# MGI-tech-bioinformatics/SuperPlus

Hardware: AMD Instinct MI355X
Metric: k-mers/s (DF createDict stage: trim + canonical k-mer count + solid filter + spectrum + adjacency) (higher is better)
Workload: dtype u64

## Files before the change

superplus_amd/csrc/dfk.hip:

```cpp
#include "../../include/dfk.h"
#include "dfk_kernels.h"

#include <algorithm>
#include <chrono>
#include <cstdarg>
#include <cstdio>
#include <cstdlib>
#include <cstring>
#include <atomic>
#include <fcntl.h>
#include <functional>
#include <new>
#include <string>
#include <sys/mman.h>
#include <sys/stat.h>
#include <unistd.h>
#include <condition_variable>
#include <memory>
#include <mutex>
#include <thread>
#include <vector>

using namespace dfk;

// ... 276 lines not shown
template <int K>
int stage_trim(dfk_ctx* c, const Inputs& in, uint64_t* n_inst)
{
    DevBuf ctr; int rc = c->alloc(ctr, 32, "trim counters"); if (rc) return rc;
    HIP_TRY(hipMemsetAsync(ctr.p, 0, 32, c->stream));
    rc = c->alloc(c->good_len, sizeof(uint32_t) * in.n_reads, "goodLens", true); if (rc) return rc;
    if (in.n_reads) {
        unsigned grid = (unsigned)std::min<uint64_t>((in.n_reads + 255) / 256, 8192);
        hipLaunchKernelGGL(HIP_KERNEL_NAME(k_trim<K>), dim3(grid), dim3(256), 0, c->stream,
                           in.pq, in.pq_off, in.pq_bytes, in.base_off, in.packed_bytes, in.read_len, in.n_reads, c->cfg.min_qual, (uint32_t*)c->good_len.p,
                           (unsigned long long*)ctr.p, (unsigned int*)((char*)ctr.p + 8),
                           (unsigned long long*)((char*)ctr.p + 16));
        HIP_TRY(hipGetLastError());
    }
    uint64_t h[3] = {0, 0, 0};
    HIP_TRY(hipMemcpyAsync(h, ctr.p, 24, hipMemcpyDeviceToHost, c->stream));
    HIP_TRY(hipStreamSynchronize(c->stream));
    c->release(ctr);
    if ((uint32_t)h[1]) return fail(DFK_E_INPUT, "malformed input: an offset table is not monotone or runs past its array, a PQVec stream is broken, or its length differs from read_len");
    if (h[2] == 0) return fail(DFK_E_NOGOOD, "Looks like your input data have almost no good bases.");
    *n_inst = h[0];
    return 0;
}

int device_scan(dfk_ctx* c, const uint64_t* in, uint64_t* out, uint64_t n)
{
    constexpr uint64_t PER = (uint64_t)SCAN_THREADS * SCAN_ITEMS;
    if (n == 0) return 0;
    const uint64_t nblk = (n + PER - 1) / PER;
    if (nblk == 1) {
        hipLaunchKernelGGL(k_scan_blocks, dim3(1), dim3(SCAN_THREADS), 0, c->stream, in, out, n, (uint64_t*)nullptr);
        HIP_TRY(hipGetLastError());
        return 0;
    }
    DevBuf sums; int rc = c->alloc(sums, nblk * 8, "scan block sums"); if (rc) return rc;
    hipLaunchKernelGGL(k_scan_blocks, dim3((unsigned)nblk), dim3(SCAN_THREADS), 0, c->stream, in, out, n, (uint64_t*)sums.p);
    HIP_TRY(hipGetLastError());
    rc = device_scan(c, (const uint64_t*)sums.p, (uint64_t*)sums.p, nblk); if (rc) return rc;
    hipLaunchKernelGGL(k_scan_add, dim3((unsigned)nblk), dim3(SCAN_THREADS), 0, c->stream, out, n, (const uint64_t*)sums.p);
    HIP_TRY(hipGetLastError());
    HIP_TRY(hipStreamSynchronize(c->stream));
    c->release(sums);
    return 0;
}

struct BucketTable {
    uint32_t log2_nb = 0;
    DevBuf acc;
    DevBuf summ;
    DevBuf classes;
    DevBuf ovf_list; uint64_t n_ovf = 0;
    DevBuf class_hist;
    std::vector<uint64_t> h_class;
    uint64_t n_records = 0, n_inst = 0;
};
struct Partition {
    DevBuf records, base, ipre, items;
    uint64_t n_records = 0, n_inst = 0, n_items = 0;
    uint64_t nb = 0;
};

template <int K>
PartParams part_params(const dfk_ctx* c, uint32_t log2_nb, uint32_t log2_world, int64_t read_id0, uint32_t sub_lo, uint32_t sub_n)
{
    const uint32_t M = c->cfg.minimizer_len;
    return PartParams{M, (uint32_t)K - M + 1, log2_nb, log2_world, read_id0, sub_lo, sub_n,
                      sweep_class_mask(sub_lo, sub_n, log2_nb - log2_world)};
}

int table_totals(dfk_ctx* c, const DevBuf& acc, uint64_t nb, uint64_t* n_records, uint64_t* n_inst)
{
    DevBuf tot; int rc = c->alloc(tot, 16, "bucket totals"); if (rc) return rc;
    HIP_TRY(hipMemsetAsync(tot.p, 0, 16, c->stream));
    hipLaunchKernelGGL(k_sum_acc, dim3(1024), dim3(256), 0, c->stream, (const unsigned long long*)acc.p, nb, (unsigned long long*)tot.p);
    HIP_TRY(hipGetLastError());
    uint64_t h[2];
    HIP_TRY(hipMemcpyAsync(h, tot.p, 16, hipMemcpyDeviceToHost, c->stream));
    HIP_TRY(hipStreamSynchronize(c->stream));
    c->release(tot);
    *n_records = h[0]; *n_inst = h[1];
    return 0;
}

struct ScanJob {
    PartParams pp; uint64_t nb = 0, n_bins = 0, ovf_cap = 0; bool by_class = false, ranged = false;
    DevBuf ovf_tmp, d_n;
    bool keyed = false; uint32_t n_cls = 0, n_sub = 0, sb = 0; uint64_t piece_reads = 0;
    ScanKeys sk{};
    DevBuf keys, keys2, fill, sub;
    std::vector<std::pair<hipEvent_t, hipEvent_t>> ev;
    ~ScanJob() { for (auto& e : ev) { (void)hipEventDestroy(e.first); (void)hipEventDestroy(e.second); } }
};

template <int K> bool scan_takes_ranges(const dfk_ctx* c) { return c->cfg.minimizer_len == 16; }

template <int K>
int scan_begin(dfk_ctx* c, const Inputs& in, uint32_t log2_world, int64_t read_id0, BucketTable* T, bool by_class, ScanJob* J)
{
    J->pp = part_params<K>(c, T->log2_nb, log2_world, read_id0, 0, 1u << (T->log2_nb - log2_world));
    J->nb = 1ull << T->log2_nb; J->by_class = by_class;
    int rc = 0;
    J->n_bins = 2ull * (PART_CLASSES << log2_world);
    if (by_class) { rc = c->alloc(T->class_hist, J->n_bins * 8, "class counters", true); if (rc) return rc; HIP_TRY(hipMemsetAsync(T->class_hist.p, 0, J->n_bins * 8, c->stream)); }
    else { rc = c->alloc(T->acc, J->nb * 8, "bucket counters", true); if (rc) return rc; }
    rc = c->alloc(T->summ, std::max<uint64_t>(1, in.n_reads) * 16, "run summaries", true); if (rc) return rc;
    rc = c->alloc(T->classes, std::max<uint64_t>(1, in.n_reads) * 4, "read bucket classes", true); if (rc) return rc;
    if (!by_class) HIP_TRY(hipMemsetAsync(T->acc.p, 0, J->nb * 8, c->stream));
    J->ovf_cap = in.n_reads / 16 + 1024;
    rc = c->alloc(J->ovf_tmp, J->ovf_cap * 4, "overflow read list (scratch)"); if (rc) return rc;
    rc = c->alloc(J->d_n, 16, "overflow read count"); if (rc) return rc;
    HIP_TRY(hipMemsetAsync(J->d_n.p, 0, 16, c->stream));
    const double runs = in.n_reads ? 1.0 + 2.0 * std::max(0.0, 4.0 * (double)in.packed_bytes / (double)in.n_reads - K + 1) / (J->pp.W + 1) : 0.0;
    J->keyed = !by_class && scan_takes_ranges<K>(c) && in.n_reads && (runs >= 3.5 || getenv("DFK_SCAN_KEY_PIECE"));
    if (J->keyed) {
        const uint32_t lb = T->log2_nb, cb = std::min<uint32_t>(6, lb);
        J->sk.ib = lb - cb; J->n_cls = 1u << cb;
        J->sb = std::min(KEY_SUB_BITS, J->sk.ib); J->n_sub = 1u << (J->sk.ib - J->sb);
        const double per_read = 1.25 * runs;
        constexpr uint64_t KEY_SCRATCH_MAX = 16ull << 30;
        const uint64_t want = 8ull * (uint64_t)(per_read * (double)in.n_reads) + 8ull * J->n_cls;
        const uint64_t room = std::min<uint64_t>(std::min(want, KEY_SCRATCH_MAX), c->largest_allocatable() / 3);
        J->sk.cap = std::max<uint64_t>(1024, room / 8 / J->n_cls);
        J->piece_reads = std::max<uint64_t>(PART_THREADS, (uint64_t)((double)(J->sk.cap * J->n_cls) / per_read));
        if (const char* e = getenv("DFK_SCAN_KEY_PIECE")) J->piece_reads = std::max<uint64_t>(1, std::min<uint64_t>(J->piece_reads, strtoull(e, nullptr, 10)));
        const uint64_t n_subs = (uint64_t)J->n_cls * J->n_sub;
        rc = c->alloc(J->keys, J->sk.cap * J->n_cls * 4, "run keys (scratch)"); if (rc) return rc;
        rc = c->alloc(J->keys2, J->sk.cap * J->n_cls * 4, "run keys by sub-slice (scratch)"); if (rc) return rc;
        rc = c->alloc(J->fill, J->n_cls * 8, "run key slice fills (scratch)"); if (rc) return rc;
        rc = c->alloc(J->sub, (3 * n_subs + 1) * 8, "run key sub-slices (scratch)"); if (rc) return rc;
        J->sk.keys = (uint32_t*)J->keys.p; J->sk.fill = (unsigned long long*)J->fill.p;
        TRACE("run keys: %u classes of %llu keys, %u sub-slices each, pieces of %llu reads", J->n_cls, (unsigned long long)J->sk.cap,
              J->n_sub, (unsigned long long)J->piece_reads);
    }
    return 0;
}

template <int K>
int scan_keys_piece(dfk_ctx* c, const Inputs& in, BucketTable* T, ScanJob* J, uint64_t r0, uint64_t r1)
{
    static const unsigned scan_blocks = getenv("DFK_SCAN_BLOCKS") ? (unsigned)atoi(getenv("DFK_SCAN_BLOCKS")) : 0;
    const unsigned cus = (unsigned)c->prop.multiProcessorCount;
    const unsigned grid = (unsigned)std::min<uint64_t>((r1 - r0 + PART_THREADS - 1) / PART_THREADS, (uint64_t)(scan_blocks ? scan_blocks : 128u) * cus);
    const uint64_t n_subs = (uint64_t)J->n_cls * J->n_sub;
    auto* cnt = (unsigned long long*)J->sub.p;
    auto* off = cnt + n_subs;
    auto* cur = off + n_subs + 1;
    HIP_TRY(hipMemsetAsync(J->fill.p, 0, J->n_cls * 8, c->stream));
    HIP_TRY(hipMemsetAsync(cnt, 0, n_subs * 8, c->stream));
    const size_t lds = SCAN_RUN_LDS + SCAN_STAGE_LDS;
    hipLaunchKernelGGL(HIP_KERNEL_NAME(k_scan_count<K, 16, true>), dim3(grid), dim3(PART_THREADS), lds, c->stream,
                       in.packed, in.packed_bytes, in.base_off, (const uint32_t*)c->good_len.p, r0, r1, J->pp,
                       (unsigned long long*)T->acc.p, (unsigned long long*)nullptr, (unsigned long long*)J->d_n.p, J->ovf_cap,
                       (uint32_t*)J->ovf_tmp.p, (uint4*)T->summ.p, (uint32_t*)T->classes.p, J->sk);
    HIP_TRY(hipGetLastError());
    const dim3 per_class(std::max(1u, 16u * cus / J->n_cls), J->n_cls);
    const uint32_t sh = 6 + J->sb;
    hipLaunchKernelGGL(k_keys_subcount, per_class, dim3(256), J->n_sub * 4, c->stream,
                       (const uint32_t*)J->keys.p, (const unsigned long long*)J->fill.p, J->sk.cap, sh, J->n_sub, cnt);
    HIP_TRY(hipGetLastError());
    hipLaunchKernelGGL(k_keys_offsets, dim3(1), dim3(1024), 0, c->stream, (const unsigned long long*)cnt, (uint32_t)n_subs, off, cur);
    HIP_TRY(hipGetLastError());
    hipLaunchKernelGGL(k_keys_partition, per_class, dim3(256), J->n_sub * 12, c->stream,
                       (const uint32_t*)J->keys.p, (const unsigned long long*)J->fill.p, J->sk.cap, sh, J->n_sub, cur, (uint32_t*)J->keys2.p);
    HIP_TRY(hipGetLastError());
    hipLaunchKernelGGL(k_keys_count, dim3((unsigned)n_subs), dim3(1024), 0, c->stream,
                       (const uint32_t*)J->keys2.p, (const unsigned long long*)off, J->sb, (unsigned long long*)T->acc.p);
    HIP_TRY(hipGetLastError());
    return 0;
}

template <int K>
int scan_range(dfk_ctx* c, const Inputs& in, BucketTable* T, ScanJob* J, uint64_t r0, uint64_t r1)
{
    if (r1 <= r0) return 0;
    const PartParams& pp = J->pp;
    const bool by_class = J->by_class;
    unsigned grid = (unsigned)((r1 - r0 + PART_THREADS - 1) / PART_THREADS);
    static const unsigned scan_blocks = getenv("DFK_SCAN_BLOCKS") ? (unsigned)atoi(getenv("DFK_SCAN_BLOCKS")) : 0;
    if (by_class) grid = std::min<unsigned>(grid, (scan_blocks ? scan_blocks : 128u) * (unsigned)c->prop.multiProcessorCount);
    else if (scan_blocks) grid = std::min<unsigned>(grid, scan_blocks * (unsigned)c->prop.multiProcessorCount);
    const size_t lds_a = (sizeof(uint32_t) + 1) * pp.W * PART_THREADS + sizeof(uint32_t) * PART_RING * PART_THREADS + (by_class ? J->n_bins * 4 : 0);
    hipEvent_t e0, e1;
    HIP_TRY(hipEventCreate(&e0)); HIP_TRY(hipEventCreate(&e1));
    J->ev.emplace_back(e0, e1);
    HIP_TRY(hipEventRecord(e0, c->stream));
    if (J->keyed) {
        for (uint64_t p0 = r0; p0 < r1; p0 += J->piece_reads) {
            int rc = scan_keys_piece<K>(c, in, T, J, p0, std::min(r1, p0 + J->piece_reads)); if (rc) return rc;
        }
    } else if (scan_takes_ranges<K>(c)) {
        const size_t lds_r = SCAN_RUN_LDS + (by_class ? J->n_bins * 4 : 0);
        hipLaunchKernelGGL(HIP_KERNEL_NAME(k_scan_count<K, 16, false>), dim3(grid), dim3(PART_THREADS), lds_r, c->stream,
                           in.packed, in.packed_bytes, in.base_off, (const uint32_t*)c->good_len.p, r0, r1, pp,
                           (unsigned long long*)T->acc.p, (unsigned long long*)T->class_hist.p, (unsigned long long*)J->d_n.p, J->ovf_cap,
                           (uint32_t*)J->ovf_tmp.p, (uint4*)T->summ.p, (uint32_t*)T->classes.p, ScanKeys{});
    } else {
        if (r0 != 0 || r1 != in.n_reads) return fail(DFK_E_STATE, "the general scan takes every read at once");
        hipLaunchKernelGGL(HIP_KERNEL_NAME(k_partition<K, false>), dim3(grid), dim3(PART_THREADS), lds_a, c->stream,
                           in.packed, in.packed_bytes, in.base_off, (const uint32_t*)c->good_len.p, in.bc,
                           (int64_t)c->cfg.ign_bc_below, in.n_reads, pp, (unsigned long long*)T->acc.p, (unsigned long long*)T->class_hist.p,
                           (unsigned long long*)J->d_n.p, J->ovf_cap, (uint4*)J->ovf_tmp.p, (uint4*)T->summ.p,
                           (const uint32_t*)nullptr, (uint64_t)0, (const uint64_t*)nullptr, (uint32_t*)T->classes.p);
    }
    HIP_TRY(hipGetLastError());
    HIP_TRY(hipEventRecord(e1, c->stream));
    return 0;
}

template <int K>
int scan_end(dfk_ctx* c, const Inputs& in, uint64_t n_inst, BucketTable* T, ScanJob* J)
{
    int rc = 0;
    T->n_ovf = 0;
    c->release(J->keys); c->release(J->keys2); c->release(J->fill); c->release(J->sub);
    if (in.n_reads) {
        HIP_TRY(hipMemcpyAsync(&T->n_ovf, J->d_n.p, 8, hipMemcpyDeviceToHost, c->stream));
        HIP_TRY(hipStreamSynchronize(c->stream));
        if (T->n_ovf > J->ovf_cap) {
            c->release(J->ovf_tmp);
            rc = c->alloc(J->ovf_tmp, in.n_reads * 4, "overflow read list (scratch)"); if (rc) return rc;
            HIP_TRY(hipMemsetAsync(J->d_n.p, 0, 16, c->stream));
            hipLaunchKernelGGL(k_select_overflow, dim3((unsigned)std::min<uint64_t>((in.n_reads + 255) / 256, 8192)), dim3(256), 0, c->stream,
                               (const uint4*)T->summ.p, in.n_reads, (uint32_t*)J->ovf_tmp.p, (unsigned long long*)J->d_n.p);
            HIP_TRY(hipGetLastError());
            HIP_TRY(hipMemcpyAsync(&T->n_ovf, J->d_n.p, 8, hipMemcpyDeviceToHost, c->stream));
            HIP_TRY(hipStreamSynchronize(c->stream));
        }
        if (T->n_ovf) {
            rc = c->alloc(T->ovf_list, T->n_ovf * 4, "overflow read list", true); if (rc) return rc;
            HIP_TRY(hipMemcpyAsync(T->ovf_list.p, J->ovf_tmp.p, T->n_ovf * 4, hipMemcpyDeviceToDevice, c->stream));
            HIP_TRY(hipStreamSynchronize(c->stream));
        }
    }
    c->release(J->ovf_tmp); c->release(J->d_n);
    HIP_TRY(hipStreamSynchronize(c->stream));
    float ms = 0;
    for (auto& e : J->ev) { float m = 0; if (hipEventElapsedTime(&m, e.first, e.second) == hipSuccess) ms += m; }
    c->st.ms_part_count = ms; c->st.reserved[6] = J->ev.size();
    TRACE("%llu of %llu reads have more than %d runs", (unsigned long long)T->n_ovf, (unsigned long long)in.n_reads, SUMMARY_RUNS);
    if (J->by_class) {
        T->h_class.assign(J->n_bins, 0);
        HIP_TRY(hipMemcpyAsync(T->h_class.data(), T->class_hist.p, J->n_bins * 8, hipMemcpyDeviceToHost, c->stream));
        HIP_TRY(hipStreamSynchronize(c->stream));
        T->n_records = T->n_inst = 0;
        for (uint64_t i = 0; i < J->n_bins / 2; ++i) { T->n_records += T->h_class[i]; T->n_inst += T->h_class[J->n_bins / 2 + i]; }
    } else { rc = table_totals(c, T->acc, J->nb, &T->n_records, &T->n_inst); if (rc) return rc; }
    TRACE("partition count pass done (%llu buckets, %llu records%s)", (unsigned long long)J->nb, (unsigned long long)T->n_records, J->ev.size() > 1 ? ", in ranges under the upload" : "");
    if (T->n_inst != n_inst)
        return fail(DFK_E_HIP, "partition count pass saw %llu instances, trim saw %llu%s",
                    (unsigned long long)T->n_inst, (unsigned long long)n_inst,
                    (n_inst - T->n_inst) % (1ull << 32) == 0 ? " (a fine bucket with 2^32 or more instances: its counter keeps 32 bits)" : "");
    c->st.n_records = T->n_records; c->st.n_buckets = J->nb;
    return 0;
}

template <int K>
int partition_count(dfk_ctx* c, const Inputs& in, uint64_t n_inst, uint32_t log2_world, int64_t read_id0, BucketTable* T, bool by_class = false)
{
    ScanJob J;
    int rc = scan_begin<K>(c, in, log2_world, read_id0, T, by_class, &J); if (rc) return rc;
    rc = scan_range<K>(c, in, T, &J, 0, in.n_reads); if (rc) return rc;
    return scan_end<K>(c, in, n_inst, T, &J);
}

int pass_tables(dfk_ctx* c, const DevBuf& acc, uint32_t log2_sub, uint32_t world, uint32_t sub_lo, uint32_t sub_n, uint64_t budget, Partition* P)
{
    P->nb = (uint64_t)world * sub_n;
    const uint64_t nb = P->nb;
    DevBuf rec, inst, flags, idx;
    int rc = c->alloc(rec, (nb + 1) * 8, "bucket record counts"); if (rc) return rc;
    rc = c->alloc(inst, (nb + 1) * 8, "bucket instance counts"); if (rc) return rc;
    rc = c->alloc(P->base, (nb + 1) * 8, "bucket bases"); if (rc) return rc;
    rc = c->alloc(P->ipre, (nb + 1) * 8, "bucket instance prefix"); if (rc) return rc;
    const unsigned g1 = (unsigned)((nb + 1 + 255) / 256);
    hipLaunchKernelGGL(k_slice, dim3(g1), dim3(256), 0, c->stream, (const unsigned long long*)acc.p, log2_sub, sub_lo, sub_n, nb,
                       (uint64_t*)rec.p, (uint64_t*)inst.p);
    HIP_TRY(hipGetLastError());
    rc = device_scan(c, (const uint64_t*)rec.p, (uint64_t*)P->base.p, nb + 1); if (rc) return rc;
    rc = device_scan(c, (const uint64_t*)inst.p, (uint64_t*)P->ipre.p, nb + 1); if (rc) return rc;
    rc = c->alloc(flags, (nb + 1) * 8, "item flags"); if (rc) return rc;
    rc = c->alloc(idx, (nb + 1) * 8, "item index"); if (rc) return rc;
    hipLaunchKernelGGL(k_item_flags, dim3(g1), dim3(256), 0, c->stream, (const uint64_t*)P->ipre.p, nb, budget, (uint64_t*)flags.p);
    HIP_TRY(hipGetLastError());
    rc = device_scan(c, (const uint64_t*)flags.p, (uint64_t*)idx.p, nb + 1); if (rc) return rc;
    uint64_t tot[3];
    HIP_TRY(hipMemcpyAsync(&tot[0], (const uint64_t*)P->base.p + nb, 8, hipMemcpyDeviceToHost, c->stream));
    HIP_TRY(hipMemcpyAsync(&tot[1], (const uint64_t*)P->ipre.p + nb, 8, hipMemcpyDeviceToHost, c->stream));
    HIP_TRY(hipMemcpyAsync(&tot[2], (const uint64_t*)idx.p + nb, 8, hipMemcpyDeviceToHost, c->stream));
    HIP_TRY(hipStreamSynchronize(c->stream));
    P->n_records = tot[0]; P->n_inst = tot[1]; P->n_items = tot[2];
    rc = c->alloc(P->items, std::max<uint64_t>(1, P->n_items) * sizeof(ItemRange), "work items"); if (rc) return rc;
    hipLaunchKernelGGL(k_item_pairs, dim3((unsigned)((nb + 255) / 256)), dim3(256), 0, c->stream, (const uint64_t*)flags.p,
                       (const uint64_t*)idx.p, nb, (ItemRange*)P->items.p);
    HIP_TRY(hipGetLastError());
    HIP_TRY(hipStreamSynchronize(c->stream));
    c->release(rec); c->release(inst); c->release(flags); c->release(idx);
// ... 1642 lines not shown
```

superplus_amd/csrc/dfk_kernels.h:

```cpp
#pragma once
#include <type_traits>
#include "dfk_device.h"

namespace dfk {

template <int K>
__global__ void __launch_bounds__(256)
k_trim(const uint8_t* __restrict__ pq, const uint64_t* __restrict__ pq_off, uint64_t pq_nbytes,
       const uint64_t* __restrict__ base_off, uint64_t packed_bytes, const uint32_t* __restrict__ read_len,
       uint64_t n_reads, uint32_t min_qual, uint32_t* __restrict__ good_len,
       unsigned long long* __restrict__ n_inst, unsigned int* __restrict__ bad,
       unsigned long long* __restrict__ sum_good)
{
    unsigned long long mine = 0, good = 0;
    bool any_bad = false;
    for (uint64_t r = (uint64_t)blockIdx.x * blockDim.x + threadIdx.x; r < n_reads; r += (uint64_t)gridDim.x * blockDim.x) {
        uint32_t gl = 0;
        uint64_t p = pq_off[r], end = pq_off[r + 1];
        uint32_t idx = 0, run = 0;
        const uint64_t b0 = base_off[r], b1 = base_off[r + 1];
        bool ok = p <= end && end <= pq_nbytes && b0 <= b1 && b1 <= packed_bytes && b1 - b0 >= ((uint64_t)read_len[r] + 3) / 4;
        if (!ok) end = p;
        while (p < end) {
            uint32_t nQs = pq[p];
// ... 267 lines not shown
                for (int k = 0; k < 8; ++k) v[k] = i0 - k >= 0 ? arr[(i0 - k) * PART_THREADS + tid] : 0u;
#pragma unroll
                for (int k = 0; k < 8; ++k) {
                    const int i = i0 - k;
                    if (i >= 0) {
                        const bool lt = v[k] < run;
                        run = lt ? v[k] : run;
                        arr[i * PART_THREADS + tid] = run;
                        if (!WRITE) { ri = lt ? (uint32_t)i : ri; sidx[i * PART_THREADS + tid] = (uint8_t)ri; }
                    }
                }
            }
            bi = 0;
        }
        if (bi + 1 < W) sfx_next = arr[(bi + 1) * PART_THREADS + tid];
    }
    close_run();
    if (!WRITE) {
        const uint64_t lo = sum_lo | (qn <= (uint32_t)SUMMARY_RUNS ? qn : SUMMARY_OVERFLOW), hi = sum_hi;
        summaries[r] = uint4{(uint32_t)lo, (uint32_t)(lo >> 32), (uint32_t)hi, (uint32_t)(hi >> 32)};
        if (read_classes) read_classes[r] = cmask;
        if (qn > (uint32_t)SUMMARY_RUNS && bucket_cur) {
            const unsigned long long at = atomicAdd(bucket_cur, 1ull);
            if (at < n_out) reinterpret_cast<uint32_t*>(records)[at] = (uint32_t)r;
        }
    }
    if (WRITE) {
        for (uint32_t e = 0; e < qn; ++e) {
            uint32_t a = queue[(2 * e) * PART_THREADS + tid], b = queue[(2 * e + 1) * PART_THREADS + tid];
            const uint64_t dst = place(b);
            if (dst != ~0ull) emit_record<K>(words, n_words, bit0, a & 0xFFFFu, a >> 16, b, gl, tag, dst, records);
        }
    }
}

template <int K, bool WRITE>
__global__ void __launch_bounds__(PART_THREADS)
k_partition(const uint8_t* __restrict__ packed, uint64_t packed_bytes, const uint64_t* __restrict__ base_off,
            const uint32_t* __restrict__ good_len, const int32_t* __restrict__ bc, int64_t ign_bc_below,
            uint64_t n_reads, PartParams pp,
            unsigned long long* __restrict__ bucket_acc,
            unsigned long long* __restrict__ class_hist,
            unsigned long long* __restrict__ bucket_cur,
            uint64_t n_out,
            uint4* __restrict__ records,
            uint4* __restrict__ summaries,
            const uint32_t* __restrict__ read_list,
            uint64_t n_list,
            const uint64_t* __restrict__ slice_base,
            uint32_t* __restrict__ read_classes)
{
    extern __shared__ uint32_t smem[];
    uint32_t* lh = nullptr;
    const uint32_t n_bins = 2u * (PART_CLASSES << pp.log2_world);
    if (!WRITE && class_hist) {
        lh = reinterpret_cast<uint32_t*>(reinterpret_cast<uint8_t*>(smem) + 5 * pp.W * PART_THREADS + 4 * PART_RING * PART_THREADS);
        for (uint32_t i = threadIdx.x; i < n_bins; i += PART_THREADS) lh[i] = 0;
        __syncthreads();
    }
    const uint64_t n_work = (WRITE && read_list) ? n_list : n_reads;
    for (uint64_t r0 = (uint64_t)blockIdx.x * PART_THREADS; r0 < n_work; r0 += (uint64_t)gridDim.x * PART_THREADS)
        partition_read<K, WRITE>(r0 + threadIdx.x, smem, lh, packed, packed_bytes, base_off, good_len, bc, ign_bc_below, n_reads, pp,
                                 bucket_acc, bucket_cur, n_out, records, summaries, read_list, n_list, slice_base, read_classes);
    if (lh) {
        __syncthreads();
        for (uint32_t i = threadIdx.x; i < n_bins; i += PART_THREADS) if (lh[i]) atomicAdd(&class_hist[i], (unsigned long long)lh[i]);
    }
}

template <int I, int N, class F>
__device__ __forceinline__ void static_for(F&& f)
{
    if constexpr (I < N) { f(std::integral_constant<int, I>{}); static_for<I + 1, N>(f); }
}

struct ScanKeys {
    uint32_t* keys;
    unsigned long long* fill;
    uint64_t cap;
    uint32_t ib;
};
constexpr int SCAN_STAGE = 1536;
constexpr uint32_t KEY_SUB_BITS = 14;
constexpr uint32_t KEY_TILE = 16384;

template <int K, int M, bool KEYS>
__global__ void __launch_bounds__(PART_THREADS)
k_scan_count(const uint8_t* __restrict__ packed, uint64_t packed_bytes, const uint64_t* __restrict__ base_off,
             const uint32_t* __restrict__ good_len, uint64_t r_first, uint64_t n_reads , PartParams pp,
             unsigned long long* __restrict__ bucket_acc, unsigned long long* __restrict__ class_hist,
             unsigned long long* __restrict__ ovf_count, uint64_t ovf_cap, uint32_t* __restrict__ ovf_list,
             uint4* __restrict__ summaries, uint32_t* __restrict__ read_classes, ScanKeys sk)
{
    constexpr int W = K - M + 1;
    constexpr uint32_t mmask = M == 16 ? 0xFFFFFFFFu : ((1u << (2 * M)) - 1u);
    constexpr uint32_t rsh = 2 * (M - 1);
    constexpr int RUNS = SUMMARY_RUNS;
    static_assert(KTraits<K>::NK_MAX < 64, "nk takes the key's six low bits");
    extern __shared__ uint32_t smem[];
    uint32_t* runb = smem;
    uint16_t* runf = reinterpret_cast<uint16_t*>(runb + RUNS * PART_THREADS);
    uint32_t* const after_runs = reinterpret_cast<uint32_t*>(runf + RUNS * PART_THREADS);
    uint32_t* lh = nullptr;
    const uint32_t n_bins = 2u * (PART_CLASSES << pp.log2_world);
    if (class_hist) {
        lh = after_runs;
        for (uint32_t i = threadIdx.x; i < n_bins; i += PART_THREADS) lh[i] = 0;
        __syncthreads();
    }
    const int tid = threadIdx.x;
    uint32_t* st_key = after_runs;
    unsigned long long* st_base = reinterpret_cast<unsigned long long*>(st_key + SCAN_STAGE);
    uint32_t* st_h = reinterpret_cast<uint32_t*>(st_base + PART_CLASSES);
    uint32_t* st_n = st_h + PART_CLASSES;
    uint8_t* st_cls = reinterpret_cast<uint8_t*>(st_n + 1);
    const uint32_t n_cls = 1u << (pp.log2_nb - sk.ib);
    if constexpr (KEYS) {
        if (tid < PART_CLASSES) st_h[tid] = 0;
        if (tid == 0) *st_n = 0;
        __syncthreads();
    }
    auto flush = [&]() {
        const uint32_t n = *st_n;
        if (tid < (int)n_cls) { const uint32_t h = st_h[tid]; if (h) st_base[tid] = atomicAdd(&sk.fill[tid], (unsigned long long)h); st_h[tid] = 0; }
        __syncthreads();
        for (uint32_t j = tid; j < n; j += PART_THREADS) {
            const uint32_t key = st_key[j], cls = st_cls[j];
            const unsigned long long at = st_base[cls] + atomicAdd(&st_h[cls], 1u);
            if (at < sk.cap) sk.keys[cls * sk.cap + at] = key;
            else atomicAdd(&bucket_acc[(cls << sk.ib) | (key >> 6)], (1ull << 32) | (key & 63u));
        }
        __syncthreads();
        if (tid < (int)n_cls) st_h[tid] = 0;
        if (tid == 0) *st_n = 0;
        __syncthreads();
    };
    const uint32_t* words = reinterpret_cast<const uint32_t*>(packed);
    const uint64_t n_words = (packed_bytes + 3) >> 2;
    const uint32_t log2_local = pp.log2_nb - pp.log2_world;
    for (uint64_t r0 = r_first + (uint64_t)blockIdx.x * PART_THREADS; r0 < n_reads; r0 += (uint64_t)gridDim.x * PART_THREADS) {
        const uint64_t r = r0 + tid;
        const uint32_t gl = r < n_reads ? good_len[r] : 0;
        const bool live = gl >= (uint32_t)K + 1;
        uint32_t qn = 0, cmask = 0;
        uint64_t sum_lo = 0, sum_hi = 0;
        if (live) {
            const uint64_t bit0 = base_off[r] * 8;
            constexpr int NW = (2 * W + 30 + 31) / 32, NA = (2 * W + 31) / 32;
            auto load = [&](uint64_t bit, uint32_t (&w)[NW]) {
                const uint64_t wi = bit >> 5;
#pragma unroll
                for (int k = 0; k < NW; ++k) {
                    const uint64_t i = wi + k;
                    const uint32_t v = words[i < n_words ? i : n_words - 1];
                    w[k] = i < n_words ? v : 0u;
                }
            };
            uint64_t nbit = bit0 + 2 * (M - 1);
            uint32_t nw[NW];
            load(nbit, nw);
            uint32_t f = 0, rc = 0;
            {
                const uint64_t wi = bit0 >> 5;
                const uint32_t w0 = words[wi < n_words ? wi : n_words - 1], w1 = words[wi + 1 < n_words ? wi + 1 : n_words - 1];
                const uint32_t pw = alignbit(wi + 1 < n_words ? w1 : 0u, wi < n_words ? w0 : 0u, (uint32_t)bit0 & 31u);
#pragma unroll
                for (int j = 0; j < M - 1; ++j) { const uint32_t b = (pw >> (2 * j)) & 3u; f = ((f << 2) | b) & mmask; rc = (rc >> 2) | ((3u - b) << rsh); }
// ... 38 lines not shown
                        Pi = newmin ? (uint32_t)bi : Pi;
                        const bool first = t0 == 0;
                        if (!first || bi == W - 1) {
                            uint32_t mv = P;
                            bool older = false;
                            if constexpr (bi != W - 1) { older = arr[bi + 1] < mv; mv = older ? arr[bi + 1] : mv; }
                            const uint32_t bucket = bucket_of(mv, pp);
                            const bool open = first || bucket != cur_b || cur_nk == (uint32_t)KTraits<K>::NK_MAX;
                            if (open && !first) close_run();
                            const uint32_t rel = (bi != W - 1 && older) ? sidx_get(bi + 1 < W ? bi + 1 : 0) - (uint32_t)bi - 1u : (uint32_t)(W - 1 - bi) + Pi;
                            cur_rel = open ? rel : cur_rel;
                            cur_nk = open ? 1u : cur_nk + 1u;
                            cur_b = open ? bucket : cur_b;
                        }
                        arr[bi] = h;
                        if (bi == W - 1) {
                            uint32_t run = h, ri = W - 1;
                            sidx_set(W - 1, W - 1);
                            static_for<0, W - 1>([&](auto j_c) {
                                constexpr int i = W - 2 - decltype(j_c)::value;
                                const bool lt = arr[i] < run; run = lt ? arr[i] : run; arr[i] = run; ri = lt ? (uint32_t)i : ri; sidx_set(i, ri);
                            });
                        }
                    }
                });
            }
            close_run();
        }
        const uint32_t mine = min(qn, (uint32_t)RUNS);
        for (uint32_t i = 0; KEYS ? __syncthreads_or(i < mine) != 0 : __ballot(i < mine) != 0ull; ++i) {
            const bool has = i < mine;
            uint32_t cb = 0, nk = 0;
            if (has) {
                cb = runb[i * PART_THREADS + tid];
                const uint64_t fld = runf[i * PART_THREADS + tid];
                nk = (uint32_t)fld & 63u;
                const uint32_t bfld = 8u + 12u * i;
                if (bfld < 64u) { sum_lo |= fld << bfld; if (bfld > 52u) sum_hi |= fld >> (64u - bfld); } else sum_hi |= fld << (bfld - 64u);
                if constexpr (!KEYS) {
                    if (lh) { const uint32_t bin = class_bin(cb, pp); atomicAdd(&lh[bin], 1u); atomicAdd(&lh[(PART_CLASSES << pp.log2_world) + bin], nk); }
                    else atomicAdd(&bucket_acc[cb], (1ull << 32) | nk);
                }
                cmask |= 1u << sweep_class_of(cb & ((1u << log2_local) - 1u), log2_local);
            }
            if constexpr (KEYS) {
                const uint64_t m = __ballot(has);
                if (m) {
                    const uint32_t rk = __builtin_amdgcn_mbcnt_hi((uint32_t)(m >> 32), __builtin_amdgcn_mbcnt_lo((uint32_t)m, 0u));
                    const int lead = __ffsll((unsigned long long)m) - 1;
                    uint32_t at = 0;
                    if (has && rk == 0) at = atomicAdd(st_n, (uint32_t)__popcll(m));
                    at = __shfl(at, lead) + rk;
                    if (has) {
                        const uint32_t cls = cb >> sk.ib;
                        st_key[at] = ((cb & ((1u << sk.ib) - 1u)) << 6) | nk;
                        st_cls[at] = (uint8_t)cls;
                        atomicAdd(&st_h[cls], 1u);
                    }
                }
                __syncthreads();
                if (*st_n > (uint32_t)(SCAN_STAGE - PART_THREADS)) flush();
            }
        }
        if (r < n_reads) {
            const uint64_t lo = sum_lo | (qn <= (uint32_t)SUMMARY_RUNS ? qn : SUMMARY_OVERFLOW);
            summaries[r] = uint4{(uint32_t)lo, (uint32_t)(lo >> 32), (uint32_t)sum_hi, (uint32_t)(sum_hi >> 32)};
            if (read_classes) read_classes[r] = cmask;
        }
        if (qn > (uint32_t)SUMMARY_RUNS) {
            const unsigned long long at = atomicAdd(ovf_count, 1ull);
            if (at < ovf_cap) ovf_list[at] = (uint32_t)r;
        }
    }
    if constexpr (KEYS) { __syncthreads(); if (*st_n) flush(); }
    if (lh) {
        __syncthreads();
        for (uint32_t i = threadIdx.x; i < n_bins; i += PART_THREADS) if (lh[i]) atomicAdd(&class_hist[i], (unsigned long long)lh[i]);
    }
}
constexpr size_t SCAN_RUN_LDS = (sizeof(uint32_t) + sizeof(uint16_t)) * SUMMARY_RUNS * PART_THREADS;
constexpr size_t SCAN_STAGE_LDS = (sizeof(uint32_t) + 1) * SCAN_STAGE + (sizeof(unsigned long long) + sizeof(uint32_t)) * PART_CLASSES + sizeof(uint32_t);
static_assert(SCAN_RUN_LDS + SCAN_STAGE_LDS <= 16384, "ten scan blocks a CU (160 KB of LDS)");

__global__ void __launch_bounds__(256)
k_keys_subcount(const uint32_t* __restrict__ keys, const unsigned long long* __restrict__ fill, uint64_t cap, uint32_t sh ,
                uint32_t n_sub, unsigned long long* __restrict__ sub_cnt)
{
    extern __shared__ uint32_t lh[];
    const uint32_t c = blockIdx.y;
    for (uint32_t i = threadIdx.x; i < n_sub; i += blockDim.x) lh[i] = 0;
    __syncthreads();
    const uint64_t n = min((uint64_t)fill[c], cap);
    const uint32_t* k = keys + c * cap;
    for (uint64_t i = (uint64_t)blockIdx.x * blockDim.x + threadIdx.x; i < n; i += (uint64_t)gridDim.x * blockDim.x) atomicAdd(&lh[k[i] >> sh], 1u);
    __syncthreads();
    for (uint32_t i = threadIdx.x; i < n_sub; i += blockDim.x) if (lh[i]) atomicAdd(&sub_cnt[(uint64_t)c * n_sub + i], (unsigned long long)lh[i]);
}

__global__ void __launch_bounds__(1024)
k_keys_offsets(const unsigned long long* __restrict__ cnt, uint32_t n, unsigned long long* __restrict__ off, unsigned long long* __restrict__ cur)
{
    __shared__ unsigned long long part[1024];
    const uint32_t tid = threadIdx.x, per = (n + 1023) / 1024;
    const uint32_t lo = min(n, tid * per), hi = min(n, lo + per);
    unsigned long long s = 0;
    for (uint32_t i = lo; i < hi; ++i) s += cnt[i];
    part[tid] = s;
    __syncthreads();
    for (uint32_t d = 1; d < 1024; d <<= 1) {
        const unsigned long long v = tid >= d ? part[tid - d] : 0ull;
        __syncthreads();
        part[tid] += v;
        __syncthreads();
    }
    unsigned long long run = part[tid] - s;
    for (uint32_t i = lo; i < hi; ++i) { off[i] = run; cur[i] = run; run += cnt[i]; }
    if (tid == 1023) off[n] = part[1023];
}

__global__ void __launch_bounds__(256)
k_keys_partition(const uint32_t* __restrict__ keys, const unsigned long long* __restrict__ fill, uint64_t cap, uint32_t sh,
                 uint32_t n_sub, unsigned long long* __restrict__ cur, uint32_t* __restrict__ out)
{
    extern __shared__ unsigned long long lds64[];
    unsigned long long* base = lds64;
    uint32_t* lh = reinterpret_cast<uint32_t*>(lds64 + n_sub);
    const uint32_t c = blockIdx.y;
    const uint64_t n = min((uint64_t)fill[c], cap);
    const uint32_t* k = keys + c * cap;
    unsigned long long* cc = cur + (uint64_t)c * n_sub;
    for (uint64_t t0 = (uint64_t)blockIdx.x * KEY_TILE; t0 < n; t0 += (uint64_t)gridDim.x * KEY_TILE) {
        const uint64_t t1 = min(n, t0 + KEY_TILE);
        for (uint32_t i = threadIdx.x; i < n_sub; i += blockDim.x) lh[i] = 0;
        __syncthreads();
        for (uint64_t i = t0 + threadIdx.x; i < t1; i += blockDim.x) atomicAdd(&lh[k[i] >> sh], 1u);
        __syncthreads();
        for (uint32_t i = threadIdx.x; i < n_sub; i += blockDim.x) { if (lh[i]) base[i] = atomicAdd(&cc[i], (unsigned long long)lh[i]); lh[i] = 0; }
        __syncthreads();
        for (uint64_t i = t0 + threadIdx.x; i < t1; i += blockDim.x) {
            const uint32_t key = k[i], s = key >> sh;
            out[base[s] + atomicAdd(&lh[s], 1u)] = key;
        }
        __syncthreads();
    }
}

__global__ void __launch_bounds__(1024)
k_keys_count(const uint32_t* __restrict__ part, const unsigned long long* __restrict__ off, uint32_t sb, unsigned long long* __restrict__ bucket_acc)
{
    __shared__ unsigned long long t[1u << KEY_SUB_BITS];
    const uint32_t s = blockIdx.x, nt = 1u << sb, m = nt - 1u;
    for (uint32_t i = threadIdx.x; i < nt; i += blockDim.x) t[i] = 0;
    __syncthreads();
    const uint64_t a = off[s], b = off[s + 1];
    for (uint64_t i = a + threadIdx.x; i < b; i += blockDim.x) {
        const uint32_t key = part[i];
        atomicAdd(&t[(key >> 6) & m], (1ull << 32) | (key & 63u));
    }
    __syncthreads();
    unsigned long long* dst = bucket_acc + ((uint64_t)s << sb);
    for (uint32_t i = threadIdx.x; i < nt; i += blockDim.x) if (t[i]) dst[i] += t[i];
}

constexpr int SLICE_READS = 16;
template <int K, bool EMIT, typename F>
__device__ __forceinline__ void for_each_run_in_pass(uint64_t r, const uint8_t* __restrict__ packed, uint64_t packed_bytes,
                                                     const uint64_t* __restrict__ base_off, const PartParams& pp,
                                                     const uint4* __restrict__ summaries, F&& f)
{
    const uint4 sm = summaries[r];
    const uint32_t n = sm.x & 15u;
    if (n == 0 || n == SUMMARY_OVERFLOW) return;
    const uint32_t* words = reinterpret_cast<const uint32_t*>(packed);
    const uint64_t n_words = (packed_bytes + 3) >> 2;
    const uint64_t bit0 = base_off[r] * 8;
    const uint32_t M = pp.M;
    const uint32_t mmask = M == 16 ? 0xFFFFFFFFu : ((1u << (2 * M)) - 1u);
    const uint64_t lo = (uint64_t)sm.x | ((uint64_t)sm.y << 32), hi = (uint64_t)sm.z | ((uint64_t)sm.w << 32);
    uint32_t s0 = 0;
#pragma unroll
    for (int i = 0; i < SUMMARY_RUNS; ++i) {
        if ((uint32_t)i < n) {
            constexpr int B0 = 8;
            const int b = B0 + 12 * i;
            const uint32_t fld = (uint32_t)(b + 12 <= 64 ? lo >> b : b >= 64 ? hi >> (b - 64) : (lo >> b) | (hi << (64 - b))) & 0xFFFu;
            const uint32_t nk = fld & 63u, rel = fld >> 6;
            const uint64_t bo = bit0 + 2ull * (s0 + rel);
            const uint64_t wi = bo >> 5;
            const uint32_t w0 = words[wi], w1 = wi + 1 < n_words ? words[wi + 1] : 0u;
            const uint32_t x = alignbit(w1, w0, (uint32_t)bo & 31u) & mmask;
            uint32_t y = __brev(x);
            y = ((y >> 1) & 0x55555555u) | ((y & 0x55555555u) << 1);
            const uint32_t fw = y >> (32 - 2 * M), rcv = ~x & mmask;
            const uint32_t bucket = bucket_of(mmer_hash(fw < rcv ? fw : rcv), pp);
            const uint32_t lb = pass_local(bucket, pp);
            if (lb != 0xFFFFFFFFu) f(s0, nk, lb, bucket >> (pp.log2_nb - pp.log2_world), bit0, (uint32_t)i + 1 == n);
            s0 += nk;
        }
    }
}

template <int K>
__global__ void __launch_bounds__(256)
k_scatter_slices(const uint8_t* __restrict__ packed, uint64_t packed_bytes, const uint64_t* __restrict__ base_off,
                 const uint32_t* __restrict__ good_len, const int32_t* __restrict__ bc, int64_t ign_bc_below,
                 uint64_t n_reads, PartParams pp, const uint4* __restrict__ summaries, const uint32_t* __restrict__ read_classes,
                 const uint64_t* __restrict__ slice_base,
                 unsigned long long* __restrict__ slice_fill,
                 uint4* __restrict__ records)
{
    __shared__ uint32_t cnt[256];
    __shared__ unsigned long long at[256];
    __shared__ uint16_t list[256 * SLICE_READS];
    __shared__ uint32_t n_list;
    const uint32_t world = 1u << pp.log2_world;
    const int lane = threadIdx.x & 63;
    const uint64_t r_block = (uint64_t)blockIdx.x * 256 * SLICE_READS;
    if (threadIdx.x < world) cnt[threadIdx.x] = 0;
    if (threadIdx.x == 0) n_list = 0;
    __syncthreads();
#pragma unroll
    for (int j = 0; j < SLICE_READS; ++j) {
        const uint32_t rel = 256u * j + threadIdx.x;
        const uint64_t r = r_block + rel;
        const bool hit = r < n_reads && (!read_classes || (read_classes[r] & pp.class_mask) != 0u);
        const unsigned long long mk = __ballot(hit);
        uint32_t w = 0;
        if (lane == 0 && mk) w = atomicAdd(&n_list, (uint32_t)__popcll(mk));
        w = __builtin_amdgcn_readfirstlane(w);
        if (hit) list[w + __popcll(mk & ((1ull << lane) - 1ull))] = (uint16_t)rel;
    }
    __syncthreads();
    const uint32_t n = n_list;
    for (uint32_t i = threadIdx.x; i < n; i += 256)
        for_each_run_in_pass<K, false>(r_block + list[i], packed, packed_bytes, base_off, pp, summaries,
                                       [&](uint32_t, uint32_t, uint32_t, uint32_t owner, uint64_t, bool) { atomicAdd(&cnt[owner], 1u); });
    __syncthreads();
    if (threadIdx.x < world) {
        const uint32_t m = cnt[threadIdx.x];
        at[threadIdx.x] = slice_base[threadIdx.x] + (m ? atomicAdd(&slice_fill[threadIdx.x], (unsigned long long)m) : 0ull);
        cnt[threadIdx.x] = 0;
    }
    __syncthreads();
    const uint32_t* words = reinterpret_cast<const uint32_t*>(packed);
// ... 1542 lines not shown
```

Baseline: 61.85 billion.

## Double-buffer run key slices and overlap key partitioning with the next scan piece

```diff
diff --git a/superplus_amd/csrc/dfk.hip b/superplus_amd/csrc/dfk.hip
--- a/superplus_amd/csrc/dfk.hip
+++ b/superplus_amd/csrc/dfk.hip
@@ -382,14 +382,21 @@
     return 0;
 }
 
+constexpr uint64_t SCAN_TAIL_READS = 32ull << 20;
 struct ScanJob {
     PartParams pp; uint64_t nb = 0, n_bins = 0, ovf_cap = 0; bool by_class = false, ranged = false;
     DevBuf ovf_tmp, d_n;
-    bool keyed = false; uint32_t n_cls = 0, n_sub = 0, sb = 0; uint64_t piece_reads = 0;
+    bool keyed = false; uint32_t n_cls = 0, n_sub = 0, sb = 0; uint64_t piece_reads = 0, tail_reads = 0;
     ScanKeys sk{};
     DevBuf keys, keys2, fill, sub;
+    uint32_t n_slices = 1; uint64_t n_pieces = 0; bool count_due = false;
+    hipEvent_t ev_scan = nullptr, ev_count = nullptr, ev_part[2] = {nullptr, nullptr};
     std::vector<std::pair<hipEvent_t, hipEvent_t>> ev;
-    ~ScanJob() { for (auto& e : ev) { (void)hipEventDestroy(e.first); (void)hipEventDestroy(e.second); } }
+    ~ScanJob()
+    {
+        for (auto& e : ev) { (void)hipEventDestroy(e.first); (void)hipEventDestroy(e.second); }
+        for (hipEvent_t e : {ev_scan, ev_count, ev_part[0], ev_part[1]}) if (e) (void)hipEventDestroy(e);
+    }
 };
 
 template <int K> bool scan_takes_ranges(const dfk_ctx* c) { return c->cfg.minimizer_len == 16; }
@@ -418,20 +425,37 @@
         J->sb = std::min(KEY_SUB_BITS, J->sk.ib); J->n_sub = 1u << (J->sk.ib - J->sb);
         const double per_read = 1.25 * runs;
         constexpr uint64_t KEY_SCRATCH_MAX = 16ull << 30;
-        const uint64_t want = 8ull * (uint64_t)(per_read * (double)in.n_reads) + 8ull * J->n_cls;
+        J->n_slices = c->stream2 && !getenv("DFK_NO_OVERLAP") ? 2 : 1;
+        const uint32_t copies = J->n_slices + 1;
+        const uint64_t want = 4ull * copies * (uint64_t)(per_read * (double)in.n_reads) + 4ull * copies * J->n_cls;
         const uint64_t room = std::min<uint64_t>(std::min(want, KEY_SCRATCH_MAX), c->largest_allocatable() / 3);
-        J->sk.cap = std::max<uint64_t>(1024, room / 8 / J->n_cls);
+        J->sk.cap = std::max<uint64_t>(1024, room / (4 * copies) / J->n_cls) & ~3ull;
         J->piece_reads = std::max<uint64_t>(PART_THREADS, (uint64_t)((double)(J->sk.cap * J->n_cls) / per_read));
         if (const char* e = getenv("DFK_SCAN_KEY_PIECE")) J->piece_reads = std::max<uint64_t>(1, std::min<uint64_t>(J->piece_reads, strtoull(e, nullptr, 10)));
+        J->tail_reads = getenv("DFK_SCAN_KEY_TAIL") ? strtoull(getenv("DFK_SCAN_KEY_TAIL"), nullptr, 10) : SCAN_TAIL_READS;
         const uint64_t n_subs = (uint64_t)J->n_cls * J->n_sub;
-        rc = c->alloc(J->keys, J->sk.cap * J->n_cls * 4, "run keys (scratch)"); if (rc) return rc;
+        rc = c->alloc(J->keys, J->n_slices * J->sk.cap * J->n_cls * 4, "run keys (scratch)"); if (rc) return rc;
         rc = c->alloc(J->keys2, J->sk.cap * J->n_cls * 4, "run keys by sub-slice (scratch)"); if (rc) return rc;
-        rc = c->alloc(J->fill, J->n_cls * 8, "run key slice fills (scratch)"); if (rc) return rc;
+        rc = c->alloc(J->fill, J->n_slices * J->n_cls * 8, "run key slice fills (scratch)"); if (rc) return rc;
         rc = c->alloc(J->sub, (3 * n_subs + 1) * 8, "run key sub-slices (scratch)"); if (rc) return rc;
-        J->sk.keys = (uint32_t*)J->keys.p; J->sk.fill = (unsigned long long*)J->fill.p;
-        TRACE("run keys: %u classes of %llu keys, %u sub-slices each, pieces of %llu reads", J->n_cls, (unsigned long long)J->sk.cap,
+        if (J->n_slices > 1)
+            for (hipEvent_t* e : {&J->ev_scan, &J->ev_count, &J->ev_part[0], &J->ev_part[1]}) HIP_TRY(hipEventCreateWithFlags(e, hipEventDisableTiming));
+        TRACE("run keys: %u x %u classes of %llu keys, %u sub-slices each, pieces of %llu reads", J->n_slices, J->n_cls, (unsigned long long)J->sk.cap,
               J->n_sub, (unsigned long long)J->piece_reads);
     }
+    return 0;
+}
+
+inline int scan_keys_count(dfk_ctx* c, BucketTable* T, ScanJob* J)
+{
+    const uint64_t n_subs = (uint64_t)J->n_cls * J->n_sub;
+    const auto* off = (const unsigned long long*)J->sub.p + n_subs;
+    if (J->n_slices > 1) HIP_TRY(hipStreamWaitEvent(c->stream, J->ev_part[(J->n_pieces - 1) & 1], 0));
+    hipLaunchKernelGGL(k_keys_count, dim3((unsigned)n_subs), dim3(1024), 0, c->stream,
+                       (const uint32_t*)J->keys2.p, off, J->sb, (unsigned long long*)T->acc.p);
+    HIP_TRY(hipGetLastError());
+    if (J->n_slices > 1) HIP_TRY(hipEventRecord(J->ev_count, c->stream));
+    J->count_due = false;
     return 0;
 }
 
@@ -442,31 +466,57 @@
     const unsigned cus = (unsigned)c->prop.multiProcessorCount;
     const unsigned grid = (unsigned)std::min<uint64_t>((r1 - r0 + PART_THREADS - 1) / PART_THREADS, (uint64_t)(scan_blocks ? scan_blocks : 128u) * cus);
     const uint64_t n_subs = (uint64_t)J->n_cls * J->n_sub;
+    const bool two = J->n_slices > 1;
+    const uint32_t sl = two ? (uint32_t)(J->n_pieces & 1) : 0;
+    hipStream_t ks = two ? c->stream2 : c->stream;
     auto* cnt = (unsigned long long*)J->sub.p;
     auto* off = cnt + n_subs;
     auto* cur = off + n_subs + 1;
-    HIP_TRY(hipMemsetAsync(J->fill.p, 0, J->n_cls * 8, c->stream));
-    HIP_TRY(hipMemsetAsync(cnt, 0, n_subs * 8, c->stream));
+    ScanKeys sk = J->sk;
+    sk.keys = (uint32_t*)J->keys.p + (uint64_t)sl * sk.cap * J->n_cls;
+    sk.fill = (unsigned long long*)J->fill.p + (uint64_t)sl * J->n_cls;
+    if (two && J->n_pieces >= 2) HIP_TRY(hipStreamWaitEvent(c->stream, J->ev_part[sl], 0));
+    HIP_TRY(hipMemsetAsync(sk.fill, 0, J->n_cls * 8, c->stream));
     const size_t lds = SCAN_RUN_LDS + SCAN_STAGE_LDS;
     hipLaunchKernelGGL(HIP_KERNEL_NAME(k_scan_count<K, 16, true>), dim3(grid), dim3(PART_THREADS), lds, c->stream,
                        in.packed, in.packed_bytes, in.base_off, (const uint32_t*)c->good_len.p, r0, r1, J->pp,
                        (unsigned long long*)T->acc.p, (unsigned long long*)nullptr, (unsigned long long*)J->d_n.p, J->ovf_cap,
-                       (uint32_t*)J->ovf_tmp.p, (uint4*)T->summ.p, (uint32_t*)T->classes.p, J->sk);
+                       (uint32_t*)J->ovf_tmp.p, (uint4*)T->summ.p, (uint32_t*)T->classes.p, sk);
     HIP_TRY(hipGetLastError());
+    if (two) {
+        HIP_TRY(hipEventRecord(J->ev_scan, c->stream));
+        if (J->count_due) { int rc = scan_keys_count(c, T, J); if (rc) return rc; }
+        HIP_TRY(hipStreamWaitEvent(ks, J->ev_scan, 0));
+        if (J->n_pieces >= 1) HIP_TRY(hipStreamWaitEvent(ks, J->ev_count, 0));
+    }
+    HIP_TRY(hipMemsetAsync(cnt, 0, n_subs * 8, ks));
     const dim3 per_class(std::max(1u, 16u * cus / J->n_cls), J->n_cls);
     const uint32_t sh = 6 + J->sb;
-    hipLaunchKernelGGL(k_keys_subcount, per_class, dim3(256), J->n_sub * 4, c->stream,
-                       (const uint32_t*)J->keys.p, (const unsigned long long*)J->fill.p, J->sk.cap, sh, J->n_sub, cnt);
+    hipLaunchKernelGGL(k_keys_subcount, per_class, dim3(256), J->n_sub * 4, ks,
+                       (const uint32_t*)sk.keys, (const unsigned long long*)sk.fill, sk.cap, sh, J->n_sub, cnt);
     HIP_TRY(hipGetLastError());
-    hipLaunchKernelGGL(k_keys_offsets, dim3(1), dim3(1024), 0, c->stream, (const unsigned long long*)cnt, (uint32_t)n_subs, off, cur);
+    hipLaunchKernelGGL(k_keys_offsets, dim3(1), dim3(1024), 0, ks, (const unsigned long long*)cnt, (uint32_t)n_subs, off, cur);
     HIP_TRY(hipGetLastError());
-    hipLaunchKernelGGL(k_keys_partition, per_class, dim3(256), J->n_sub * 12, c->stream,
-                       (const uint32_t*)J->keys.p, (const unsigned long long*)J->fill.p, J->sk.cap, sh, J->n_sub, cur, (uint32_t*)J->keys2.p);
+    hipLaunchKernelGGL(k_keys_partition, per_class, dim3(256), J->n_sub * 12, ks,
+                       (const uint32_t*)sk.keys, (const unsigned long long*)sk.fill, sk.cap, sh, J->n_sub, cur, (uint32_t*)J->keys2.p);
     HIP_TRY(hipGetLastError());
-    hipLaunchKernelGGL(k_keys_count, dim3((unsigned)n_subs), dim3(1024), 0, c->stream,
-                       (const uint32_t*)J->keys2.p, (const unsigned long long*)off, J->sb, (unsigned long long*)T->acc.p);
-    HIP_TRY(hipGetLastError());
-    return 0;
+    if (two) HIP_TRY(hipEventRecord(J->ev_part[sl], ks));
+    ++J->n_pieces; J->count_due = true;
+    if (!two) return scan_keys_count(c, T, J);
+    return 0;
+}
+
+inline std::vector<uint64_t> scan_piece_sizes(const ScanJob* J, uint64_t n, bool last)
+{
+    std::vector<uint64_t> tail;
+    uint64_t t_sum = 0;
+    if (last && J->n_slices > 1 && J->tail_reads)
+        for (uint64_t t = J->tail_reads; t < J->piece_reads && t_sum + t < n; t *= 2) { tail.push_back(t); t_sum += t; }
+    std::vector<uint64_t> v;
+    const uint64_t body = n - t_sum, nb = (body + J->piece_reads - 1) / J->piece_reads;
+    for (uint64_t i = 0, at = 0; i < nb; ++i) { const uint64_t e = body * (i + 1) / nb; v.push_back(e - at); at = e; }
+    v.insert(v.end(), tail.rbegin(), tail.rend());
+    return v;
 }
 
 template <int K>
@@ -485,9 +535,12 @@
     J->ev.emplace_back(e0, e1);
     HIP_TRY(hipEventRecord(e0, c->stream));
     if (J->keyed) {
-        for (uint64_t p0 = r0; p0 < r1; p0 += J->piece_reads) {
-            int rc = scan_keys_piece<K>(c, in, T, J, p0, std::min(r1, p0 + J->piece_reads)); if (rc) return rc;
-        }
+        uint64_t p0 = r0;
+        for (uint64_t m : scan_piece_sizes(J, r1 - r0, r1 == in.n_reads)) {
+            int rc = scan_keys_piece<K>(c, in, T, J, p0, p0 + m); if (rc) return rc;
+            p0 += m;
+        }
+        if (r1 == in.n_reads && J->count_due) { int rc = scan_keys_count(c, T, J); if (rc) return rc; }
     } else if (scan_takes_ranges<K>(c)) {
         const size_t lds_r = SCAN_RUN_LDS + (by_class ? J->n_bins * 4 : 0);
         hipLaunchKernelGGL(HIP_KERNEL_NAME(k_scan_count<K, 16, false>), dim3(grid), dim3(PART_THREADS), lds_r, c->stream,
@@ -512,6 +565,7 @@
 {
     int rc = 0;
     T->n_ovf = 0;
+    if (J->count_due) { rc = scan_keys_count(c, T, J); if (rc) return rc; }
     c->release(J->keys); c->release(J->keys2); c->release(J->fill); c->release(J->sub);
     if (in.n_reads) {
         HIP_TRY(hipMemcpyAsync(&T->n_ovf, J->d_n.p, 8, hipMemcpyDeviceToHost, c->stream));
diff --git a/superplus_amd/csrc/dfk_kernels.h b/superplus_amd/csrc/dfk_kernels.h
--- a/superplus_amd/csrc/dfk_kernels.h
+++ b/superplus_amd/csrc/dfk_kernels.h
@@ -373,7 +373,7 @@
 };
 constexpr int SCAN_STAGE = 1536;
 constexpr uint32_t KEY_SUB_BITS = 14;
-constexpr uint32_t KEY_TILE = 16384;
+constexpr uint32_t KEY_TILE = 4096;
 
 template <int K, int M, bool KEYS>
 __global__ void __launch_bounds__(PART_THREADS)
@@ -578,6 +578,35 @@
 constexpr size_t SCAN_STAGE_LDS = (sizeof(uint32_t) + 1) * SCAN_STAGE + (sizeof(unsigned long long) + sizeof(uint32_t)) * PART_CLASSES + sizeof(uint32_t);
 static_assert(SCAN_RUN_LDS + SCAN_STAGE_LDS <= 16384, "ten scan blocks a CU (160 KB of LDS)");
 
+constexpr int KEY_VECS = 4;
+static_assert(KEY_TILE == 256u * 4u * KEY_VECS, "a tile is KEY_VECS 16-byte vectors per thread of a 256-thread block");
+__device__ __forceinline__ uint32_t key_vec_n(uint64_t t0, uint64_t t1, int j)
+{
+    const uint64_t i = t0 + ((uint64_t)j * 256u + threadIdx.x) * 4u;
+    return i < t1 ? (uint32_t)min((uint64_t)4, t1 - i) : 0u;
+}
+__device__ __forceinline__ void key_tile_load(const uint32_t* __restrict__ k, uint64_t t0, uint64_t t1, uint4 (&v)[KEY_VECS])
+{
+#pragma unroll
+    for (int j = 0; j < KEY_VECS; ++j) {
+        const uint64_t i = t0 + ((uint64_t)j * 256u + threadIdx.x) * 4u;
+        v[j] = i < t1 ? *reinterpret_cast<const uint4*>(k + i) : make_uint4(0u, 0u, 0u, 0u);
+    }
+}
+template <typename F>
+__device__ __forceinline__ void key_tile_each(uint64_t t0, uint64_t t1, const uint4 (&v)[KEY_VECS], F&& f)
+{
+#pragma unroll
+    for (int j = 0; j < KEY_VECS; ++j) {
+        const uint32_t m = key_vec_n(t0, t1, j);
+        if (m > 0) f(v[j].x);
+        if (m > 1) f(v[j].y);
+        if (m > 2) f(v[j].z);
+        if (m > 3) f(v[j].w);
+        __builtin_amdgcn_sched_barrier(0);
+    }
+}
+
 __global__ void __launch_bounds__(256)
 k_keys_subcount(const uint32_t* __restrict__ keys, const unsigned long long* __restrict__ fill, uint64_t cap, uint32_t sh ,
                 uint32_t n_sub, unsigned long long* __restrict__ sub_cnt)
@@ -588,7 +617,12 @@
     __syncthreads();
     const uint64_t n = min((uint64_t)fill[c], cap);
     const uint32_t* k = keys + c * cap;
-    for (uint64_t i = (uint64_t)blockIdx.x * blockDim.x + threadIdx.x; i < n; i += (uint64_t)gridDim.x * blockDim.x) atomicAdd(&lh[k[i] >> sh], 1u);
+    for (uint64_t t0 = (uint64_t)blockIdx.x * KEY_TILE; t0 < n; t0 += (uint64_t)gridDim.x * KEY_TILE) {
+        const uint64_t t1 = min(n, t0 + KEY_TILE);
+        uint4 v[KEY_VECS];
+        key_tile_load(k, t0, t1, v);
+        key_tile_each(t0, t1, v, [&](uint32_t key) { atomicAdd(&lh[key >> sh], 1u); });
+    }
     __syncthreads();
     for (uint32_t i = threadIdx.x; i < n_sub; i += blockDim.x) if (lh[i]) atomicAdd(&sub_cnt[(uint64_t)c * n_sub + i], (unsigned long long)lh[i]);
 }
@@ -627,16 +661,17 @@
     unsigned long long* cc = cur + (uint64_t)c * n_sub;
     for (uint64_t t0 = (uint64_t)blockIdx.x * KEY_TILE; t0 < n; t0 += (uint64_t)gridDim.x * KEY_TILE) {
         const uint64_t t1 = min(n, t0 + KEY_TILE);
+        uint4 v[KEY_VECS];
+        key_tile_load(k, t0, t1, v);
         for (uint32_t i = threadIdx.x; i < n_sub; i += blockDim.x) lh[i] = 0;
         __syncthreads();
-        for (uint64_t i = t0 + threadIdx.x; i < t1; i += blockDim.x) atomicAdd(&lh[k[i] >> sh], 1u);
+        key_tile_each(t0, t1, v, [&](uint32_t key) { atomicAdd(&lh[key >> sh], 1u); });
         __syncthreads();
         for (uint32_t i = threadIdx.x; i < n_sub; i += blockDim.x) { if (lh[i]) base[i] = atomicAdd(&cc[i], (unsigned long long)lh[i]); lh[i] = 0; }
         __syncthreads();
-        for (uint64_t i = t0 + threadIdx.x; i < t1; i += blockDim.x) {
-            const uint32_t key = k[i], s = key >> sh;
-            out[base[s] + atomicAdd(&lh[s], 1u)] = key;
-        }
+        uint32_t sh2 = sh;
+        asm volatile("" : "+s"(sh2));
+        key_tile_each(t0, t1, v, [&](uint32_t key) { const uint32_t s = key >> sh2; out[base[s] + atomicAdd(&lh[s], 1u)] = key; });
         __syncthreads();
     }
 }
@@ -655,7 +690,7 @@
     }
     __syncthreads();
     unsigned long long* dst = bucket_acc + ((uint64_t)s << sb);
-    for (uint32_t i = threadIdx.x; i < nt; i += blockDim.x) if (t[i]) dst[i] += t[i];
+    for (uint32_t i = threadIdx.x; i < nt; i += blockDim.x) if (t[i]) atomicAdd(&dst[i], t[i]);
 }
 
 constexpr int SLICE_READS = 16;
```

Result: faster. 64.76 billion (median of 6 runs) (+4.7%).
